# IRMVLab/EfficientLO-Net

Hardware: AMD Instinct MI355X
Metric: frame-pairs/sec (KITTI 64x1800 range image) (higher is better)
Workload: dtype f32 (1x1 convolutions as 3 fp16-MFMA products of hi/lo-split fp32 operands, fp32 accumulate)

## Files before the change

efficientlo-net_amd/csrc/elo_features.hip:

```cpp
#include <type_traits>
#include "elo_common.h"
#include "elo_project_device.h"

namespace elo {
namespace {

constexpr int ROWS_PER_BLOCK = ELO_BLOCK / ELO_WAVE;

__device__ __forceinline__ long row_of_wave(long total_rows)
{
    const long r = (long)xcd_tile(blockIdx.x, gridDim.x) * ROWS_PER_BLOCK + threadIdx.x / ELO_WAVE;
    return r < total_rows ? r : -1;
}

inline unsigned grid_for_rows(long rows) { return (unsigned)((rows + ROWS_PER_BLOCK - 1) / ROWS_PER_BLOCK); }

constexpr int STAGE_ROWS = 64;

__device__ __forceinline__ void stream_out(const float *tile, float *__restrict__ dst, long first_row, long rows, int CT)
{
    const long valid = (rows - first_row < STAGE_ROWS ? rows - first_row : STAGE_ROWS) * CT;
    float *o = dst + first_row * CT;
    const long vec = valid >> 2;
    for (long i = threadIdx.x; i < vec; i += ELO_BLOCK)
// ... 698 lines not shown
};

struct RowsByBeams {
    const float *mid;
    int half;
    __device__ __forceinline__ int cell(float at, float z, float r, int H, int W, float az_res) const
    {
        const float PI_F = 3.14159265358979323846f;
        const float c = (PI_F - at) / az_res;
        int col = c != c ? 0 : (int)c;
        const float s = z / r;
        int row = 0;
        for (int step = half; step >= 1; step >>= 1) row += !(s >= mid[row + step - 1]) ? step : 0;
        row = row > H - 1 ? H - 1 : row;
        col = col < 0 ? 0 : col > W - 1 ? W - 1 : col;
        return row * W + col;
    }
};

template <class Rows>
__device__ __forceinline__ void bin_point_by(float x, float y, float z, long i, int b, int H, int W, float az_res, const Rows &rows,
                                             const ProjScratch &ps)
{
    const float r = sqrtf(x * x + y * y + z * z);
    const float at = atan2f(y, x);
    const int cell = rows.cell(at, z, r, H, W, az_res);
    const unsigned rb = __float_as_uint(r);
    ps.cell_of[i] = cell;
    ps.rbits[i] = rb;
    if (rb == 0) {
        const int flag = b * ZFLAGS + zero_kind(at);
        const unsigned long long zeros = __ballot(1);
        const int leader = __ffsll((long long)zeros) - 1;
        if ((int)(threadIdx.x & 63) == leader || flag != __shfl(flag, leader)) ps.zflag[flag] = 0u;
        return;
    }
    unsigned *slot = ps.minr + (long)b * H * W + cell;
    if (__hip_atomic_load(slot, __ATOMIC_RELAXED, __HIP_MEMORY_SCOPE_AGENT) > rb) atomicMin(slot, rb);
}

__device__ __forceinline__ void bin_point(float x, float y, float z, long i, int b, int H, int W, float az_res, float vert_res,
                                          float vert_off, const ProjScratch &ps)
{
    bin_point_by(x, y, z, i, b, H, W, az_res, RowsByFormula{vert_res, vert_off}, ps);
}

__device__ __forceinline__ void warp_cell_point(const elo_warp_project_args &a, long i, int b, const float *q, const float *t,
                                                const ProjScratch &ps)
{
    float x = a.xyz[i * 3 + 0], y = a.xyz[i * 3 + 1], z = a.xyz[i * 3 + 2];
    if (q) {
        const bool keep = !(x == 0.0f && y == 0.0f && z == 0.0f);
        const float q0 = q[0], q1 = q[1], q2 = q[2], q3 = q[3];
        const float v0 = q0 * 0.0f - q1 * x - q2 * y - q3 * z;
        const float v1 = q0 * x + q1 * 0.0f + q2 * z - q3 * y;
        const float v2 = q0 * y - q1 * z + q2 * 0.0f + q3 * x;
        const float v3 = q0 * z + q1 * y - q2 * x + q3 * 0.0f;
        const float n2 = q0 * q0 + q1 * q1 + q2 * q2 + q3 * q3 + 1e-10f;
        const float i0 = q0 / n2, i1 = -q1 / n2, i2 = -q2 / n2, i3 = -q3 / n2;
        const float w1 = v0 * i1 + v1 * i0 + v2 * i3 - v3 * i2;
        const float w2 = v0 * i2 - v1 * i3 + v2 * i0 + v3 * i1;
        const float w3 = v0 * i3 + v1 * i2 - v2 * i1 + v3 * i0;
        const float k = keep ? 1.0f : 0.0f;
        x = (w1 + t[0]) * k; y = (w2 + t[1]) * k; z = (w3 + t[2]) * k;
        a.warped[i * 3 + 0] = x; a.warped[i * 3 + 1] = y; a.warped[i * 3 + 2] = z;
    }
    bin_point(x, y, z, i, b, a.H, a.W, a.az_res, a.vert_res, a.vert_off, ps);
}

__device__ __forceinline__ void hamilton(const float *a, const float *b, float *r)
{
    r[0] = a[0] * b[0] - a[1] * b[1] - a[2] * b[2] - a[3] * b[3];
    r[1] = a[0] * b[1] + a[1] * b[0] + a[2] * b[3] - a[3] * b[2];
    r[2] = a[0] * b[2] - a[1] * b[3] + a[2] * b[0] + a[3] * b[1];
    r[3] = a[0] * b[3] + a[1] * b[2] - a[2] * b[1] + a[3] * b[0];
}

__device__ __forceinline__ void normalise_q(const float *q, float *o)
{
    const float n = sqrtf(q[0] * q[0] + q[1] * q[1] + q[2] * q[2] + q[3] * q[3] + 1e-10f) + 1e-10f;
    for (int i = 0; i < 4; ++i) o[i] = q[i] / n;
}

#ifdef ELO_POSE_CLOCK
__device__ unsigned long long g_pose_clock[4 * 8 + 1];
#define POSE_STAMP(i) do { if (blockIdx.x == 0 && blockIdx.y == 0 && threadIdx.x == 0) {                                    \
        if ((i) == 0) pose_slot = (int)(g_pose_clock[32]++ % 4);                                                          \
        g_pose_clock[pose_slot * 8 + (i)] = __builtin_readcyclecounter(); } } while (0)
#else
#define POSE_STAMP(i) do { } while (0)
#endif

template <int BLOCK>
__global__ __launch_bounds__(BLOCK) void pose_head_kernel(const elo_pose_head_args a, const int parts,
                                                          const elo_warp_project_args w, const int with_warp)
{
    extern __shared__ float sm[];
    float *feat = sm, *big = sm + a.C, *head = big + a.hidden;
    const int b = blockIdx.y, tid = threadIdx.x;
    const SvPartials s = sv_partials(a.scratch, gridDim.y, a.C);
#ifdef ELO_POSE_CLOCK
    int pose_slot = 0;
#endif
    POSE_STAMP(0);
    constexpr int HEAD_C = 64;
    const bool model_head = a.C == HEAD_C && a.hidden == BLOCK;
    float wb[HEAD_C], wq[4], wt[3], bias_big = 0.0f;
    auto request_weights = [&]() {
        const int j = tid;
#pragma unroll
        for (int c = 0; c < HEAD_C; ++c) wb[c] = a.W_big[(size_t)c * a.hidden + j];
#pragma unroll
        for (int o = 0; o < 4; ++o) wq[o] = a.W_q[(size_t)j * 4 + o];
#pragma unroll
        for (int o = 0; o < 3; ++o) wt[o] = a.W_t[(size_t)j * 3 + o];
        bias_big = a.b_big[j];
    };
    float *mpart = head + 8 + 8 * (BLOCK / ELO_WAVE);
    if (model_head) request_weights();
    const int c = tid & 63, q = tid >> 6;
    float M = -INFINITY, D = 0.0f, A = 0.0f;
    if (c < a.C) {
        auto trips = [&](auto mine) {
            constexpr int MINE = decltype(mine)::value;
            for (int i0 = q; i0 < parts; i0 += 4 * MINE) {
                float m_[MINE], d_[MINE], a_[MINE];
#pragma unroll
                for (int u = 0; u < MINE; ++u) {
                    const int i = i0 + 4 * u;
                    const size_t at = ((size_t)b * ELO_SV_MAX_PARTS + (i < parts ? i : 0)) * a.C + c;
                    m_[u] = s.mx[at]; a_[u] = s.acc[at];
                    d_[u] = i < parts ? s.den[at] : 0.0f;
                }
#pragma unroll
                for (int u = 0; u < MINE; ++u) {
                    if (d_[u] == 0.0f) continue;
                    if (m_[u] > M) { const float sc = exp_acc(M - m_[u]); D = D * sc + d_[u]; A = A * sc + a_[u]; M = m_[u]; }
                    else { const float sc = exp_acc(m_[u] - M); D += d_[u] * sc; A += a_[u] * sc; }
                }
            }
        };
        if (parts <= 64) trips(std::integral_constant<int, 16>());
        else trips(std::integral_constant<int, 32>());
    }
    POSE_STAMP(1);
    mpart[(0 * 4 + q) * 64 + c] = M; mpart[(1 * 4 + q) * 64 + c] = D; mpart[(2 * 4 + q) * 64 + c] = A;
    __syncthreads();
    if (tid < 64) {
        float MM = -INFINITY;
        for (int i = 0; i < 4; ++i) MM = fmaxf(MM, mpart[(0 * 4 + i) * 64 + tid]);
        float DD = 0.0f, AA = 0.0f;
        for (int i = 0; i < 4; ++i) {
            if (mpart[(1 * 4 + i) * 64 + tid] == 0.0f) continue;
            const float sc = exp_acc(mpart[(0 * 4 + i) * 64 + tid] - MM);
            DD += mpart[(1 * 4 + i) * 64 + tid] * sc; AA += mpart[(2 * 4 + i) * 64 + tid] * sc;
        }
        if (tid < a.C) feat[tid] = DD > 0.0f ? AA / DD : 0.0f;
    }
    for (int c2 = 64 + tid; c2 < a.C; c2 += blockDim.x) feat[c2] = sv_merge(s, b, c2, a.C, parts);

    __syncthreads();
    POSE_STAMP(2);
    if (model_head) {
        float v = bias_big;
#pragma unroll
        for (int c = 0; c < HEAD_C; ++c) v += feat[c] * wb[c];
        big[tid] = v;
    } else {
        for (int j = tid; j < a.hidden; j += blockDim.x) {
            float v = a.b_big[j];
#pragma unroll 16
            for (int c = 0; c < a.C; ++c) v += feat[c] * a.W_big[(size_t)c * a.hidden + j];
            big[j] = v;
        }
    }
    __syncthreads();
    POSE_STAMP(3);
    {
        float part[7] = {0, 0, 0, 0, 0, 0, 0};
        if (model_head) {
            const float bj = big[tid];
#pragma unroll
            for (int o = 0; o < 4; ++o) part[o] += bj * wq[o];
#pragma unroll
            for (int o = 0; o < 3; ++o) part[4 + o] += bj * wt[o];
        } else {
            for (int j = tid; j < a.hidden; j += blockDim.x) {
                const float bj = big[j];
#pragma unroll
                for (int o = 0; o < 4; ++o) part[o] += bj * a.W_q[(size_t)j * 4 + o];
#pragma unroll
                for (int o = 0; o < 3; ++o) part[4 + o] += bj * a.W_t[(size_t)j * 3 + o];
            }
        }
#pragma unroll
        for (int o = 0; o < 7; ++o)
            for (int d = 32; d >= 1; d >>= 1) part[o] += __shfl_xor(part[o], d, ELO_WAVE);
        float *wsum = head + 8;
        if ((tid & 63) == 0)
            for (int o = 0; o < 7; ++o) wsum[(tid >> 6) * 8 + o] = part[o];
        __syncthreads();
        if (tid < 7) {
            float v = tid < 4 ? a.b_q[tid] : a.b_t[tid - 4];
            for (int w = 0; w < (int)(blockDim.x >> 6); ++w) v += wsum[w * 8 + tid];
            head[tid] = v;
        }
    }
    __syncthreads();
    POSE_STAMP(4);
    if (tid == 0) {
        float q_det[4], q[4], t[3], qn[4];
        normalise_q(head, q_det);
        const float *t_det = head + 4;
        if (a.q_coarse) {
            const float *qc = a.q_coarse + b * 4, *tc = a.t_coarse + b * 3;
            const float tq[4] = {0.0f, tc[0], tc[1], tc[2]};
            float v[4], w[4], inv[4];
            hamilton(q_det, tq, v);
            const float n2 = q_det[0] * q_det[0] + q_det[1] * q_det[1] + q_det[2] * q_det[2] + q_det[3] * q_det[3] + 1e-10f;
            inv[0] = q_det[0] / n2; inv[1] = -q_det[1] / n2; inv[2] = -q_det[2] / n2; inv[3] = -q_det[3] / n2;
            hamilton(v, inv, w);
            hamilton(q_det, qc, q);
            for (int i = 0; i < 3; ++i) t[i] = w[i + 1] + t_det[i];
        } else {
            for (int i = 0; i < 4; ++i) q[i] = q_det[i];
            for (int i = 0; i < 3; ++i) t[i] = t_det[i];
        }
        normalise_q(q, qn);
        if (blockIdx.x == 0) {
            for (int i = 0; i < 4; ++i) { a.q[b * 4 + i] = q[i]; a.q_norm[b * 4 + i] = qn[i]; }
            for (int i = 0; i < 3; ++i) a.t[b * 3 + i] = t[i];
            if (a.pose7) {
                float *row = a.pose7 + b * 7;
                if (a.pose7_slots > 1 && a.pose7_cursor) {
                    const unsigned at = a.pose7_cursor[b];
                    a.pose7_cursor[b] = at + 1u;
                    row += (size_t)(at % (unsigned)a.pose7_slots) * a.batch * 7;
                }
                for (int i = 0; i < 4; ++i) row[i] = qn[i];
                for (int i = 0; i < 3; ++i) row[4 + i] = t[i];
            }
        }
        if (with_warp) {
            for (int i = 0; i < 4; ++i) head[8 + i] = q[i];
            for (int i = 0; i < 3; ++i) head[12 + i] = t[i];
        }
    }
    POSE_STAMP(5);
    if (a.next_orders.pool && blockIdx.x == 0 && blockIdx.y == 0) perm_refresh_block(a.next_orders);
    POSE_STAMP(6);
    if (!with_warp) return;
    __syncthreads();
    const long n = (long)blockIdx.x * blockDim.x + tid;
    if (n < w.npoints) {
        warp_cell_point(w, (long)b * w.npoints + n, b, head + 8, head + 12,
                        proj_scratch(w.scratch, (size_t)w.batch * w.H * w.W, w.batch, (size_t)w.batch * w.npoints));
    }
    POSE_STAMP(7);
}

__global__ __launch_bounds__(ELO_BLOCK) void project_init_kernel(unsigned *minr, float *out_xyz, unsigned *out_feat,
                                                                 size_t cells, int C, int images)
{
    const size_t n_xyz = cells * 3, n_feat = cells * (size_t)C, total = cells + n_xyz + n_feat;
    for (size_t i = (size_t)blockIdx.x * blockDim.x + threadIdx.x; i < (size_t)images * ZFLAGS; i += (size_t)gridDim.x * blockDim.x)
        minr[cells + i] = 0x7f7f7f7fu;
    for (size_t i = (size_t)blockIdx.x * blockDim.x + threadIdx.x; i < total; i += (size_t)gridDim.x * blockDim.x) {
        if (i < cells) minr[i] = 0x7f7f7f7fu;
        else if (i < cells + n_xyz) out_xyz[i - cells] = 0.0f;
        else out_feat[i - cells - n_xyz] = 0u;
    }
}

__global__ __launch_bounds__(ELO_BLOCK) void warp_cell_kernel(const elo_warp_project_args a, const ProjScratch ps)
{
    const long total = (long)a.batch * a.npoints;
    for (long i = (long)blockIdx.x * blockDim.x + threadIdx.x; i < total; i += (long)gridDim.x * blockDim.x) {
        const int b = point_batch(i, a.npoints);
        warp_cell_point(a, i, b, a.q ? a.q + b * 4 : nullptr, a.q ? a.t + b * 3 : nullptr, ps);
    }
// ... 606 lines not shown
```

efficientlo-net_amd/csrc/elo_fused.hip:

```cpp
#include "elo_group_device.h"
#include "elo_project_device.h"
#include <atomic>
#include <cstdlib>
#include <type_traits>

namespace elo {
namespace {

typedef float f32x4 __attribute__((ext_vector_type(4)));
typedef _Float16 half4 __attribute__((ext_vector_type(4)));
typedef _Float16 half2v __attribute__((ext_vector_type(2)));

constexpr int FUSED_BLOCK = 256;
constexpr int FUSED_WAVES = 4;
__device__ __forceinline__ int ftid() { return (int)(threadIdx.x & (FUSED_BLOCK - 1)); }

constexpr int MODE_SPLIT = 0;
constexpr int MODE_HALF = 1;
constexpr int MODE_CHECKED = 2;

__device__ unsigned long long g_range_violations;
__device__ unsigned long long g_range_snapshot;
__global__ void range_take_kernel() { g_range_snapshot = atomicExch(&g_range_violations, 0ull); }

// ... 1016 lines not shown
        seg_store<TILE, MODE>(act, S, 0, w0, f16, r0, row_of, all, bad);
        if (w1) seg_store<TILE, MODE>(act, S, w0, w1, f16, r1, row_of, all, bad);
        if (w2) seg_store<TILE, MODE>(act, S, w0 + w1, w2, f16, r2, row_of, all, bad);
        zero_cols<TILE, MODE>(act, S, CT, CTp);
    } else {
        for (int e = tid; e < TILE * CTp; e += FUSED_BLOCK) {
            const int row = small_div(e, CTp), ch = e - row * CTp;
            const long gr = first + row;
            float v = 0.0f;
            if (gr < end && ch < CT) {
                v = ch < w0 ? feat_load(a.src[0], gr * w0 + ch, f16)
                  : ch < w0 + w1 ? feat_load(a.src[1], gr * w1 + (ch - w0), f16)
                                 : feat_load(a.src[2], gr * w2 + (ch - w0 - w1), f16);
            }
            act_put<MODE>(act, row * S + ch, v, bad);
        }
    }
    __syncthreads();
    const int N = a.layers[a.n_layers - 1].N;
    const bool two = a.n_layers2 > 0;
    for (int l = 0; l < a.n_layers; ++l)
        dense<TILE, MODE>(act, S, 0, a.layers[l],
                          l == a.n_layers - 1 ? LayerOut{two || keep_final ? 0 : -1, !two && keep_final ? 1 : 0, a.out, first, end, f16} : to_tile(0), bad);
    if (!two) return;
    const int wb = a.w_before, wa = a.w_after, CT2 = N + wb + wa;
    if ((N & 3) == 0 && (wb == 0 || seg_ok(a.before, wb, TILE, f16)) && (wa == 0 || seg_ok(a.after, wa, TILE, f16))) {
        uint4 rb[SEG_ITEMS], ra[SEG_ITEMS];
        if (wb) seg_load<TILE>(rb, a.before, wb, f16, row_of);
        if (wa) seg_load<TILE>(ra, a.after, wa, f16, row_of);
        if (wb) seg_store<TILE, MODE>(act, S, N, wb, f16, rb, row_of, all, bad);
        if (wa) seg_store<TILE, MODE>(act, S, N + wb, wa, f16, ra, row_of, all, bad);
    } else {
        for (int e = tid; e < TILE * (wb + wa); e += FUSED_BLOCK) {
            const int row = small_div(e, wb + wa), ch = e - row * (wb + wa);
            const long gr = first + row;
            const long grc = gr < end ? gr : end - 1;
            const float v = ch < wb ? feat_load(a.before, grc * wb + ch, f16) : feat_load(a.after, grc * wa + (ch - wb), f16);
            act_put<MODE>(act, row * S + N + ch, gr < end ? v : 0.0f, bad);
        }
    }
    zero_cols<TILE, MODE>(act, S, CT2, ceil16(CT2));
    __syncthreads();
    for (int l = 0; l < a.n_layers2; ++l)
        dense<TILE, MODE>(act, S, 0, a.layers2[l],
                          l == a.n_layers2 - 1 ? LayerOut{keep_final ? 0 : -1, keep_final ? 1 : 0, a.out2, first, end, f16} : to_tile(0), bad);
}

template <int TILE, int MODE>
__global__ __launch_bounds__(FUSED_BLOCK, TILE == 32 ? ELO_TILE32_WAVES : ELO_TILE_WAVES) void mlp_kernel(const JobPair<elo_mlp_args> jobs, const int S)
{
    const elo_mlp_args &a = jobs.job[blockIdx.y];
    extern __shared__ __align__(16) float lds[];
    unsigned bad = 0;
    {
        const elo_mlp_args &j0 = jobs.job[0];
        clear_projection(ProjectionClear{j0.clear_scratch, j0.clear_xyz, (unsigned *)j0.clear_feat, j0.clear_cells,
                                         j0.feat_dtype == ELO_F16 ? j0.clear_C / 2 : j0.clear_C, j0.clear_images});
    }
    const long first = (long)xcd_tile(blockIdx.x, gridDim.x) * TILE;
    if (first >= a.rows) return;
    mlp_tile<TILE, MODE>(a, lds, S, first, a.rows, false, bad);
    report_violations<MODE>(bad, a.range_counter);
}

template <int TILE, int MODE, bool PAIR>
__global__ __launch_bounds__(PAIR ? 2 * FUSED_BLOCK : FUSED_BLOCK, TILE == 32 ? 4 : ELO_TILE_WAVES)
void mlp_sv_kernel(const JobPair<elo_mlp_args> jobs, const int S, const int tiles_pb)
{
    constexpr int C = 64;
    const int group = PAIR ? __builtin_amdgcn_readfirstlane(threadIdx.x >> 8) : 0;
    const elo_mlp_args &j0 = jobs.job[0];
    const elo_mlp_args &a = jobs.job[group];
    extern __shared__ __align__(16) float lds[];
    const int tile_words = TILE * S;
    float *act = lds + group * tile_words;
    float *staged = lds + (PAIR ? 2 : 1) * tile_words;
    unsigned bad = 0;
    clear_projection(ProjectionClear{j0.clear_scratch, j0.clear_xyz, (unsigned *)j0.clear_feat, j0.clear_cells,
                                     j0.feat_dtype == ELO_F16 ? j0.clear_C / 2 : j0.clear_C, j0.clear_images});
    const unsigned tile = xcd_tile(blockIdx.x, gridDim.x);
    const int b = (int)(tile / (unsigned)tiles_pb), t = (int)(tile - (unsigned)b * (unsigned)tiles_pb);
    const long first = (long)b * j0.sv_npoints + (long)t * TILE, end = (long)(b + 1) * j0.sv_npoints;
    const int f16 = j0.feat_dtype == ELO_F16;
    const int vr = threadIdx.x < TILE ? (int)threadIdx.x : 0;
    const long vrow = first + vr < end ? first + vr : end - 1;
    const float px = j0.sv_xyz[vrow * 3 + 0], py = j0.sv_xyz[vrow * 3 + 1], pz = j0.sv_xyz[vrow * 3 + 2];
    constexpr int STAGE = PAIR ? 1 : TILE / 16;
    uint4 held[STAGE];
    if constexpr (!PAIR) {
#pragma unroll
        for (int u = 0; u < STAGE; ++u) {
            const int e = (int)threadIdx.x + u * FUSED_BLOCK, fr = e >> 4, q = e & 15;
            const long grow = first + fr < end ? first + fr : end - 1;
            if (f16) { const uint2 h = reinterpret_cast<const uint2 *>(j0.sv_feature)[grow * (C / 4) + q]; held[u] = uint4{h.x, h.y, 0u, 0u}; }
            else held[u] = reinterpret_cast<const uint4 *>(j0.sv_feature)[grow * (C / 4) + q];
        }
    }
    mlp_tile<TILE, MODE>(a, act, S, first, end, true, bad);
    report_violations<MODE>(bad, a.range_counter);
    if constexpr (!PAIR) {
#pragma unroll
        for (int u = 0; u < STAGE; ++u) {
            const int e = (int)threadIdx.x + u * FUSED_BLOCK, fr = e >> 4, q = e & 15;
            float4 v;
            if (f16) {
                const half2v h0 = __builtin_bit_cast(half2v, held[u].x), h1 = __builtin_bit_cast(half2v, held[u].y);
                v = float4{(float)h0.x, (float)h0.y, (float)h1.x, (float)h1.y};
            } else {
                v = __builtin_bit_cast(float4, held[u]);
            }
            *reinterpret_cast<float4 *>(staged + fr * C + 4 * q) = v;
        }
        __syncthreads();
    }
    if (threadIdx.x >= C) return;
    const unsigned long long okm = __ballot((threadIdx.x < TILE) & (first + vr < end) & !((px == 0.0f) & (py == 0.0f) & (pz == 0.0f)));
    const int c = threadIdx.x;
    const float *logit = lds + c, *value = PAIR ? lds + tile_words + c : staged + c;
    const int vs = PAIR ? S : C;
    float M = -INFINITY, D = 0.0f, A = 0.0f;
#pragma unroll
    for (int r0 = 0; r0 < TILE; r0 += 16) {
        float l[16], v[16];
#pragma unroll
        for (int r = 0; r < 16; ++r) { l[r] = logit[(r0 + r) * S]; v[r] = value[(r0 + r) * vs]; }
        const unsigned ok = (unsigned)(okm >> r0) & 0xffffu;
        float bm = -INFINITY;
#pragma unroll
        for (int r = 0; r < 16; ++r) bm = (ok >> r & 1u) ? fmaxf(bm, l[r]) : bm;
        if (bm > -INFINITY) {
            float d16 = 0.0f, a16 = 0.0f;
#pragma unroll
            for (int r = 0; r < 16; ++r) {
                const float e = (ok >> r & 1u) ? exp_acc(l[r] - bm) : 0.0f;
                d16 += e;
                a16 += e * v[r];
            }
            const float m2 = fmaxf(M, bm), s0 = exp_acc(M - m2), s1 = exp_acc(bm - m2);
            D = D * s0 + d16 * s1;
            A = A * s0 + a16 * s1;
            M = m2;
        }
    }
    float *sc = j0.sv_scratch;
    const size_t n = (size_t)(gridDim.x / (unsigned)tiles_pb) * ELO_SV_MAX_PARTS * C;
    const size_t at = ((size_t)b * ELO_SV_MAX_PARTS + t) * C + c;
    sc[at] = M; sc[n + at] = D; sc[2 * n + at] = A;
}

__host__ __device__ __forceinline__ int cv1_feat_cols(int C)
{
    const int kp = (10 + 2 * C + 15) & ~15;
    return kp > 2 * C + 16 ? kp : 2 * C + 16;
}

__device__ __forceinline__ elo_dense kernarg_dense(size_t byte_offset)
{
    static_assert(sizeof(elo_dense) == 48, "three 16-byte scalar loads");
    typedef const __attribute__((address_space(4))) char *KernargBytes;
    typedef unsigned int Quad __attribute__((ext_vector_type(4)));
    typedef const __attribute__((address_space(4))) Quad *KernargQuads;
    KernargBytes p = (KernargBytes)__builtin_amdgcn_kernarg_segment_ptr() + byte_offset;
    asm volatile("" : "+s"(p));
    KernargQuads q = reinterpret_cast<KernargQuads>(p);
    struct Raw { Quad a, b, c; } raw = {q[0], q[1], q[2]};
    return __builtin_bit_cast(elo_dense, raw);
}
#define CV1_LAYER(field) kernarg_dense(offsetof(elo_cv1_args, field))

template <int TILE, int MODE, bool GROUP = true>
__device__ __forceinline__ void cv1_tile(const elo_cv1_args &a, const int S, float *lds, unsigned block, unsigned nblocks)
{
    float *act = lds;
    const TileMeta meta = tile_meta(lds, TILE, S);
    const int tid = threadIdx.x;
    const int K = a.K, P = TILE / K, C = a.C, f16 = a.feat_dtype == ELO_F16;
    unsigned bad = 0;
    const long total_points = (long)a.batch * a.npoints;
    const long first_point = (long)xcd_tile(block, nblocks) * P;
    if (first_point >= total_points) return;
    CV1_STAMP(0);
    if (GROUP && a.group.random_hw) {
        int *lds_off = reinterpret_cast<int *>(act);
        unsigned *scratch = reinterpret_cast<unsigned *>(lds_off + ((a.group.kernel_h * a.group.kernel_w + 3) & ~3));
        group_tile<TILE, true>(meta, lds_off, scratch, a.group, first_point, total_points, a.npoints, P, K, a.xyz1, a.H2,
                               a.W2, nullptr, a.xyz2, a.H2, a.W2, nullptr);
    } else {
        load_meta<TILE>(meta, first_point, total_points, P, K, a.idx, a.mask, a.H2, a.W2);
        __syncthreads();
    }
    CV1_STAMP(1);
    const int F = 128, G = F + 2 * C;
    {
        auto cell_of = [&](int row) { return (long)meta.cell[row]; };
        auto centre_of = [&](int row) { return meta.cell[row] >= 0 ? first_point + small_div(row, K) : -1L; };
        uint4 r1[SEG_ITEMS], r2[SEG_ITEMS];
        seg_load<TILE>(r1, a.feat1, C, f16, centre_of);
        seg_load<TILE>(r2, a.feat2, C, f16, cell_of);
        GeoRow gr;
        const bool grow = tid < TILE;
        const int gcell = grow ? meta.cell[tid] : -1;
        if (grow) gr = geo_load(a.xyz1 + (gcell >= 0 ? first_point + small_div(tid, K) : 0) * 3, a.xyz2 + (long)(gcell >= 0 ? gcell : 0) * 3);
        seg_store<TILE, MODE>(act, S, F, C, f16, r1, centre_of, [](int) { return true; }, bad);
        seg_store<TILE, MODE>(act, S, F + C, C, f16, r2, cell_of, [&](int row) { return meta.mask[row] != 0.0f; }, bad);
        if (grow) geo_store<MODE>(act, tid * S + G, gr, meta.mask[tid], gcell >= 0, bad);
        zero_cols<TILE, MODE>(act, S, G + 16, F + cv1_feat_cols(C));
    }
    Pre<Sub<TILE, 128>::TPW> p128;
    Pre<Sub<TILE, 64>::TPW> p64;
    const elo_dense cv0 = CV1_LAYER(cv0);
    prefetch<TILE, Sub<TILE, 128>::TPW, MODE>(cv0, p128);
    __syncthreads();
    CV1_STAMP(2);
    const elo_dense cv1 = CV1_LAYER(cv1);
    dense_pf<TILE, 128, 64, MODE>(act, S, F, to_tile(0), cv0, p128, &cv1, &p64, bad);
    CV1_STAMP(3);
    const elo_dense cv2 = CV1_LAYER(cv2);
    dense_pf<TILE, 64, 64, MODE>(act, S, 0, to_tile(0), cv1, p64, &cv2, &p64, bad);
    CV1_STAMP(4);
    const elo_dense cv_xyz = CV1_LAYER(cv_xyz);
    dense_pf<TILE, 64, 64, MODE>(act, S, 0, to_tile(0), cv2, p64, &cv_xyz, &p64, bad);
    CV1_STAMP(5);
    const elo_dense sum_cv0 = CV1_LAYER(sum_cv0);
    dense_pf<TILE, 64, 128, MODE>(act, S, G, to_tile(64), cv_xyz, p64, &sum_cv0, &p128, bad);
    CV1_STAMP(6);
// ... 1532 lines not shown
    ELO_REQUIRE(!a->clear_scratch || a->clear_cells * (a->clear_C > 3 ? a->clear_C : 3) < (1l << 31), who, "clear_* side job: more than 2^31 words");
    ELO_REQUIRE(a->n_layers2 >= 0 && a->n_layers2 <= ELO_MAX_CHAIN, who, "0..3 second-stage layers");
    if (a->n_layers2 > 0) {
        ELO_REQUIRE(a->out2 && a->w_before >= 0 && a->w_after >= 0 && (a->before || a->w_before == 0) &&
                    (a->after || a->w_after == 0), who, "incomplete second stage");
        ELO_REQUIRE(width % 4 == 0, who, "a second stage needs a first-stage output width that is a multiple of 4");
        width += a->w_before + a->w_after;
        for (int l = 0; l < a->n_layers2; ++l) {
            if (int rc = check_dense(a->layers2[l], width, 0, who, "mlp stage 2")) return rc;
            width = a->layers2[l].N;
        }
    }
    return ELO_OK;
}

static int mlp_cols(const elo_mlp_args *a, int in_width)
{
    int cols = chain_cols(a->layers, a->n_layers, in_width);
    if (a->n_layers2 > 0) {
        const int n1 = a->layers[a->n_layers - 1].N, in2 = a->w_before + n1 + a->w_after;
        const int c2 = chain_cols(a->layers2, a->n_layers2, in2);
        cols = cols > c2 ? cols : c2;
    }
    return cols;
}

static bool mlp_chain_regime(long rows, bool pair, int batch_hint, int mode)
{
#ifdef ELO_DENSE_F32
    (void)rows; (void)pair; (void)batch_hint; (void)mode;
    return false;
#else
    return (mode == MODE_SPLIT || mode == MODE_HALF) && cv1_rr_on() && rows * (pair ? 2 : 1) >= mlp_rr_rows(batch_hint);
#endif
}

struct MlpPlan { int S, mode, C; bool t16, chain; int sv_tiles; size_t sv_lds; };

static int plan_mlp(const elo_mlp_args *a, const elo_mlp_args *b, MlpPlan *p, const char *who)
{
    int in_width = 0, in_width_b = 0;
    if (int rc = check_mlp(a, who, &in_width)) return rc;
    if (b) {
        if (int rc = check_mlp(b, who, &in_width_b)) return rc;
        bool same = a->rows == b->rows && in_width == in_width_b && a->n_layers == b->n_layers &&
                    a->n_layers2 == b->n_layers2 && a->w_before == b->w_before && a->w_after == b->w_after &&
                    a->feat_dtype == b->feat_dtype;
        for (int l = 0; same && l < a->n_layers; ++l) same = a->layers[l].N == b->layers[l].N;
        for (int l = 0; same && l < a->n_layers2; ++l) same = a->layers2[l].N == b->layers2[l].N;
        if (!same) return fail(ELO_ERR_ARG, "%s: the two jobs of a paired launch must have the same shape", who);
    }
    if (b && b->clear_scratch) return fail(ELO_ERR_ARG, "%s: the clear_* side job belongs to the first job of a pair", who);
    if (b && (b->sv_scratch || b->sv_feature)) return fail(ELO_ERR_ARG, "%s: the sv_* fields belong to the first job of a pair", who);
    p->S = row_stride(mlp_cols(a, in_width));
    const long u32 = (a->rows + 31) / 32;
    p->mode = 0;
    if (int rc = pair_products_mode(who, &p->mode, a->n_layers, a->n_layers2, a->layers, a->layers2, b ? b->layers : nullptr,
                                    b ? b->layers2 : nullptr))
        return rc;
    p->t16 = small_tile(u32 * (b ? 2 : 1), 1);
    p->chain = false;
    p->C = a->n_sources == 2 ? a->src_width[1] : 0;
#ifndef ELO_DENSE_F32
    {
        const int C = p->C;
        const auto aligned16 = [](const elo_mlp_args *j) {
            return ((uintptr_t)j->src[0] | (uintptr_t)j->src[1] | (uintptr_t)j->before | (uintptr_t)j->after | (uintptr_t)j->out |
                    (uintptr_t)j->out2) % 16 == 0;
        };
        const bool aligned = aligned16(a) && (!b || aligned16(b));
        p->chain = a->n_sources == 2 && a->src_width[0] == 64 &&
                   (C == 16 || C == 32 || C == 64) && a->n_layers == 2 && a->layers[0].N == 128 && a->layers[1].N == 64 && a->n_layers2 == 2 &&
                   a->layers2[0].N == 128 && a->layers2[1].N == 64 && a->w_before == C && a->w_after == 64 && aligned &&
                   mlp_chain_regime(a->rows, b != nullptr, a->batch_hint, p->mode);
    }
#endif
    p->sv_tiles = 0;
    p->sv_lds = 0;
    const int final_n = a->n_layers2 > 0 ? a->layers2[a->n_layers2 - 1].N : a->layers[a->n_layers - 1].N;
    if (!p->chain && final_n == 64 && a->sv_npoints > 0 && a->rows > 0 && a->rows % a->sv_npoints == 0) {
        const bool t16 = small_tile((a->rows / a->sv_npoints) * (((long)a->sv_npoints + 31) / 32), 1);
        const int tile = t16 ? 16 : 32, groups = b ? 2 : 1;
        const long tiles = ((long)a->sv_npoints + tile - 1) / tile;
        const size_t lds = sizeof(float) * ((size_t)groups * tile * p->S + (b ? 0 : (size_t)tile * 64));
        if (tiles <= ELO_SV_MAX_PARTS && lds <= 64 * 1024) {
            p->sv_tiles = (int)tiles;
            p->sv_lds = lds;
            p->t16 = t16;
        }
    }
    return ELO_OK;
}

extern "C" int elo_mlp_sv_parts(const elo_mlp_args *a, const elo_mlp_args *b)
{
    MlpPlan p;
    if (plan_mlp(a, b, &p, "elo_mlp_sv_parts")) return 0;
    return p.sv_tiles;
}

extern "C" int elo_mlp_fused2(const elo_mlp_args *a, const elo_mlp_args *b, elo_stream_t stream)
{
    const char *who = "elo_mlp_fused";
    MlpPlan plan;
    if (int rc = plan_mlp(a, b, &plan, who)) return rc;
    if (a->rows == 0)
        return a->clear_scratch || a->sv_scratch ? fail(ELO_ERR_ARG, "%s: a clear_* / sv_* side job needs rows to ride on", who) : ELO_OK;
    const int S = plan.S, mode = plan.mode;
    const bool t16 = plan.t16;
    const long u32 = (a->rows + 31) / 32, u16 = (a->rows + 15) / 16;
    JobPair<elo_mlp_args> pair;
    pair.job[0] = *a;
    pair.job[1] = b ? *b : *a;
    if (a->sv_scratch) {
        if (!plan.sv_tiles)
            return fail(ELO_ERR_ARG, "%s: sv_scratch is set but this launch cannot compute softmax_valid's partial sums "
                                     "(elo_mlp_sv_parts returns 0: chain-kernel regime, final width != 64, rows %% sv_npoints != 0 or too many tiles)", who);
        if (!a->sv_xyz) return fail(ELO_ERR_ARG, "%s: sv_scratch without sv_xyz", who);
        if ((b != nullptr) == (a->sv_feature != nullptr))
            return fail(ELO_ERR_ARG, "%s: a paired launch takes its features from job b (sv_feature NULL), a single launch from sv_feature", who);
        if (!b && ((uintptr_t)a->sv_feature & 15)) return fail(ELO_ERR_ARG, "%s: unaligned sv_feature", who);
        const size_t lds = plan.sv_lds;
        const dim3 grid((unsigned)(a->rows / a->sv_npoints) * (unsigned)plan.sv_tiles);
        hipStream_t s = (hipStream_t)stream;
#define CALL_SV(T_, M_)                                                                                                         \
        do {                                                                                                                    \
            if (b) hipLaunchKernelGGL((mlp_sv_kernel<T_, M_, true>), grid, dim3(2 * FUSED_BLOCK), lds, s, pair, S, plan.sv_tiles); \
            else hipLaunchKernelGGL((mlp_sv_kernel<T_, M_, false>), grid, dim3(FUSED_BLOCK), lds, s, pair, S, plan.sv_tiles);     \
        } while (0)
#define CALL_SV_T(M_, t16_) do { if (t16_) CALL_SV(16, M_); else CALL_SV(32, M_); } while (0)
        ELO_PICK_MODE(mode, CALL_SV_T, t16);
#undef CALL_SV_T
#undef CALL_SV
        ++g_sv_ride_launches;
        return check_launch(who);
    }
    const size_t lds = tile_lds_bytes(t16 ? 16 : 32, S);
#ifndef ELO_DENSE_F32
    if (plan.chain) {
        const dim3 rgrid((unsigned)((a->rows + RR_ROWS - 1) / RR_ROWS), b ? 2u : 1u);
        const bool f16 = a->feat_dtype == ELO_F16;
#define CALL(k) ELO_LAUNCH_RR(k, rgrid, (hipStream_t)stream, pair)
        ELO_PICK_RR_C(mlp2_rr_kernel, plan.C, f16, mode, CALL);
#undef CALL
        ++g_rr_launches[3];
        return check_launch(who);
    }
#endif
    const dim3 grid((unsigned)(t16 ? u16 : u32), b ? 2u : 1u);
    hipStream_t s = (hipStream_t)stream;
#define CALL(k) hipLaunchKernelGGL(k, grid, dim3(FUSED_BLOCK), lds, s, pair, S)
    ELO_PICK(mlp_kernel, t16, mode, CALL);
#undef CALL
    return check_launch(who);
}

extern "C" int elo_mlp_fused(const elo_mlp_args *a, elo_stream_t stream) { return elo_mlp_fused2(a, nullptr, stream); }

static int check_cv_features(const char *who, int C, int f16, std::initializer_list<const void *> tensors)
{
    const int per = f16 ? 8 : 4;
    if (C % per != 0) return fail(ELO_ERR_LIMIT, "%s: C = %d must be a multiple of %d (%s feature storage)", who, C, per, f16 ? "fp16" : "fp32");
    if (32 * (C / per) > SEG_ITEMS * FUSED_BLOCK) return fail(ELO_ERR_LIMIT, "%s: C = %d too wide for the tile gather", who, C);
    for (const void *p : tensors)
        if ((uintptr_t)p & 15) return fail(ELO_ERR_ARG, "%s: feature tensors must be 16-byte aligned", who);
    return ELO_OK;
}
// ... 261 lines not shown
```

Baseline: 12690.

## Parallelize softmax-pool tile reduction across waves and restructure pose-head merge

In the fused MLP softmax-pool epilogue, every wave now reduces a strided subset of tile rows per channel and writes (max, denom, acc) partials to LDS. One wave then merges those partials, where before a single wave walked every row serially. The pose head's partial merge first computes a block-wide channel max through LDS so each part is scaled once, with no running online rescaling. Its wave sums now use DPP row-rotate steps instead of a full shfl_xor tree. This adds an extra barrier and more LDS per block, which could affect occupancy.

```diff
diff --git a/efficientlo-net_amd/csrc/elo_features.hip b/efficientlo-net_amd/csrc/elo_features.hip
--- a/efficientlo-net_amd/csrc/elo_features.hip
+++ b/efficientlo-net_amd/csrc/elo_features.hip
@@ -804,6 +804,21 @@
     for (int i = 0; i < 4; ++i) o[i] = q[i] / n;
 }
 
+__device__ __forceinline__ float wave_sum_xor_tree(float v)
+{
+    const auto add = [](float x, float y) { return x + y; };
+    const auto ror = [](float x, auto ctrl) {
+        const int u = (int)__float_as_uint(x);
+        return x + __uint_as_float((unsigned)__builtin_amdgcn_update_dpp(u, u, decltype(ctrl)::value, 0xf, 0xf, false));
+    };
+    v = bfly<32>(v, add);
+    v = bfly<16>(v, add);
+    v = bfly<8>(v, add);
+    v = ror(v, std::integral_constant<int, 0x124>());
+    v = ror(v, std::integral_constant<int, 0x122>());
+    return ror(v, std::integral_constant<int, 0x121>());
+}
+
 #ifdef ELO_POSE_CLOCK
 __device__ unsigned long long g_pose_clock[4 * 8 + 1];
 #define POSE_STAMP(i) do { if (blockIdx.x == 0 && blockIdx.y == 0 && threadIdx.x == 0) {                                    \
@@ -840,44 +855,82 @@
     };
     float *mpart = head + 8 + 8 * (BLOCK / ELO_WAVE);
     if (model_head) request_weights();
-    const int c = tid & 63, q = tid >> 6;
-    float M = -INFINITY, D = 0.0f, A = 0.0f;
-    if (c < a.C) {
-        auto trips = [&](auto mine) {
-            constexpr int MINE = decltype(mine)::value;
-            for (int i0 = q; i0 < parts; i0 += 4 * MINE) {
-                float m_[MINE], d_[MINE], a_[MINE];
-#pragma unroll
-                for (int u = 0; u < MINE; ++u) {
-                    const int i = i0 + 4 * u;
-                    const size_t at = ((size_t)b * ELO_SV_MAX_PARTS + (i < parts ? i : 0)) * a.C + c;
-                    m_[u] = s.mx[at]; a_[u] = s.acc[at];
-                    d_[u] = i < parts ? s.den[at] : 0.0f;
-                }
-#pragma unroll
-                for (int u = 0; u < MINE; ++u) {
-                    if (d_[u] == 0.0f) continue;
-                    if (m_[u] > M) { const float sc = exp_acc(M - m_[u]); D = D * sc + d_[u]; A = A * sc + a_[u]; M = m_[u]; }
-                    else { const float sc = exp_acc(m_[u] - M); D += d_[u] * sc; A += a_[u] * sc; }
-                }
+    const int c = tid & 63, q = tid >> 6, cc = c < a.C ? c : a.C - 1;
+    const auto slot = [&](int i) { return ((size_t)b * ELO_SV_MAX_PARTS + (i < parts ? i : 0)) * a.C + cc; };
+    const auto channel_max = [&](float mine) {
+        mpart[q * 64 + c] = mine;
+        __syncthreads();
+        return fmaxf(fmaxf(mpart[0 * 64 + c], mpart[1 * 64 + c]), fmaxf(mpart[2 * 64 + c], mpart[3 * 64 + c]));
+    };
+    float D = 0.0f, A = 0.0f;
+    const auto held = [&](auto mine) {
+        constexpr int MINE = decltype(mine)::value;
+        float m_[MINE], d_[MINE], a_[MINE];
+#pragma unroll
+        for (int u = 0; u < MINE; ++u) {
+            const int i = q + 4 * u;
+            m_[u] = s.mx[slot(i)];
+            d_[u] = i < parts ? s.den[slot(i)] : 0.0f;
+        }
+#pragma unroll
+        for (int u = 0; u < MINE; ++u) a_[u] = s.acc[slot(q + 4 * u)];
+        float lm = -INFINITY;
+#pragma unroll
+        for (int u = 0; u < MINE; ++u) {
+            const bool live = d_[u] != 0.0f;
+            m_[u] = live ? m_[u] : -INFINITY; a_[u] = live ? a_[u] : 0.0f;
+            lm = fmaxf(lm, m_[u]);
+        }
+        const float MM = channel_max(lm);
+#pragma unroll
+        for (int u = 0; u < MINE; ++u) {
+            const float sc = exp_acc(m_[u] - MM);
+            D += d_[u] * sc;
+            A += a_[u] * sc;
+        }
+    };
+    const auto reread = [&]() {
+        constexpr int MAXES = 32, SUMS = 16;
+        float lm = -INFINITY;
+        for (int i0 = q; i0 < parts; i0 += 4 * MAXES) {
+            float m_[MAXES], d_[MAXES];
+#pragma unroll
+            for (int u = 0; u < MAXES; ++u) {
+                const int i = i0 + 4 * u;
+                m_[u] = s.mx[slot(i)];
+                d_[u] = i < parts ? s.den[slot(i)] : 0.0f;
             }
-        };
-        if (parts <= 64) trips(std::integral_constant<int, 16>());
-        else trips(std::integral_constant<int, 32>());
-    }
+#pragma unroll
+            for (int u = 0; u < MAXES; ++u) lm = d_[u] != 0.0f ? fmaxf(lm, m_[u]) : lm;
+        }
+        const float MM = channel_max(lm);
+        for (int i0 = q; i0 < parts; i0 += 4 * SUMS) {
+            float m_[SUMS], d_[SUMS], a_[SUMS];
+#pragma unroll
+            for (int u = 0; u < SUMS; ++u) {
+                const int i = i0 + 4 * u;
+                m_[u] = s.mx[slot(i)]; a_[u] = s.acc[slot(i)];
+                d_[u] = i < parts ? s.den[slot(i)] : 0.0f;
+            }
+#pragma unroll
+            for (int u = 0; u < SUMS; ++u) {
+                const bool live = d_[u] != 0.0f;
+                const float sc = exp_acc((live ? m_[u] : -INFINITY) - MM);
+                D += d_[u] * sc;
+                A += (live ? a_[u] : 0.0f) * sc;
+            }
+        }
+    };
+    if (parts <= 64) held(std::integral_constant<int, 16>());
+    else if (parts <= 128) held(std::integral_constant<int, 32>());
+    else reread();
     POSE_STAMP(1);
-    mpart[(0 * 4 + q) * 64 + c] = M; mpart[(1 * 4 + q) * 64 + c] = D; mpart[(2 * 4 + q) * 64 + c] = A;
+    mpart[(1 * 4 + q) * 64 + c] = D; mpart[(2 * 4 + q) * 64 + c] = A;
     __syncthreads();
-    if (tid < 64) {
-        float MM = -INFINITY;
-        for (int i = 0; i < 4; ++i) MM = fmaxf(MM, mpart[(0 * 4 + i) * 64 + tid]);
-        float DD = 0.0f, AA = 0.0f;
-        for (int i = 0; i < 4; ++i) {
-            if (mpart[(1 * 4 + i) * 64 + tid] == 0.0f) continue;
-            const float sc = exp_acc(mpart[(0 * 4 + i) * 64 + tid] - MM);
-            DD += mpart[(1 * 4 + i) * 64 + tid] * sc; AA += mpart[(2 * 4 + i) * 64 + tid] * sc;
-        }
-        if (tid < a.C) feat[tid] = DD > 0.0f ? AA / DD : 0.0f;
+    if (tid < 64 && tid < a.C) {
+        const float *dp = mpart + 1 * 4 * 64 + tid, *ap = mpart + 2 * 4 * 64 + tid;
+        const float DD = (dp[0 * 64] + dp[1 * 64]) + (dp[2 * 64] + dp[3 * 64]), AA = (ap[0 * 64] + ap[1 * 64]) + (ap[2 * 64] + ap[3 * 64]);
+        feat[tid] = DD > 0.0f ? AA / DD : 0.0f;
     }
     for (int c2 = 64 + tid; c2 < a.C; c2 += blockDim.x) feat[c2] = sv_merge(s, b, c2, a.C, parts);
 
@@ -916,8 +969,7 @@
             }
         }
 #pragma unroll
-        for (int o = 0; o < 7; ++o)
-            for (int d = 32; d >= 1; d >>= 1) part[o] += __shfl_xor(part[o], d, ELO_WAVE);
+        for (int o = 0; o < 7; ++o) part[o] = wave_sum_xor_tree(part[o]);
         float *wsum = head + 8;
         if ((tid & 63) == 0)
             for (int o = 0; o < 7; ++o) wsum[(tid >> 6) * 8 + o] = part[o];
diff --git a/efficientlo-net_amd/csrc/elo_fused.hip b/efficientlo-net_amd/csrc/elo_fused.hip
--- a/efficientlo-net_amd/csrc/elo_fused.hip
+++ b/efficientlo-net_amd/csrc/elo_fused.hip
@@ -1122,7 +1122,10 @@
     const int b = (int)(tile / (unsigned)tiles_pb), t = (int)(tile - (unsigned)b * (unsigned)tiles_pb);
     const long first = (long)b * j0.sv_npoints + (long)t * TILE, end = (long)(b + 1) * j0.sv_npoints;
     const int f16 = j0.feat_dtype == ELO_F16;
-    const int vr = threadIdx.x < TILE ? (int)threadIdx.x : 0;
+    constexpr int NW = (PAIR ? 2 : 1) * FUSED_WAVES, RPW = TILE / NW;
+    float *part = staged + (PAIR ? 0 : TILE * C);
+    const int lane = (int)(threadIdx.x & 63u), wave = __builtin_amdgcn_readfirstlane((int)(threadIdx.x >> 6));
+    const int vr = lane < TILE ? lane : 0;
     const long vrow = first + vr < end ? first + vr : end - 1;
     const float px = j0.sv_xyz[vrow * 3 + 0], py = j0.sv_xyz[vrow * 3 + 1], pz = j0.sv_xyz[vrow * 3 + 2];
     constexpr int STAGE = PAIR ? 1 : TILE / 16;
@@ -1153,34 +1156,37 @@
         }
         __syncthreads();
     }
+    const unsigned long long okm = __ballot((lane < TILE) & (first + vr < end) & !((px == 0.0f) & (py == 0.0f) & (pz == 0.0f)));
+    {
+        const float *logit = lds + lane, *value = PAIR ? lds + tile_words + lane : staged + lane;
+        const int vs = PAIR ? S : C;
+        float l[RPW], v[RPW];
+#pragma unroll
+        for (int k = 0; k < RPW; ++k) { l[k] = logit[(wave + k * NW) * S]; v[k] = value[(wave + k * NW) * vs]; }
+        float bm = -INFINITY;
+#pragma unroll
+        for (int k = 0; k < RPW; ++k) bm = (okm >> (wave + k * NW) & 1ull) ? fmaxf(bm, l[k]) : bm;
+        float d = 0.0f, a_ = 0.0f;
+#pragma unroll
+        for (int k = 0; k < RPW; ++k) {
+            const float e = (okm >> (wave + k * NW) & 1ull) ? exp_acc(l[k] - bm) : 0.0f;
+            d += e;
+            a_ += e * v[k];
+        }
+        part[(wave * 3 + 0) * C + lane] = bm; part[(wave * 3 + 1) * C + lane] = d; part[(wave * 3 + 2) * C + lane] = a_;
+    }
+    __syncthreads();
     if (threadIdx.x >= C) return;
-    const unsigned long long okm = __ballot((threadIdx.x < TILE) & (first + vr < end) & !((px == 0.0f) & (py == 0.0f) & (pz == 0.0f)));
     const int c = threadIdx.x;
-    const float *logit = lds + c, *value = PAIR ? lds + tile_words + c : staged + c;
-    const int vs = PAIR ? S : C;
     float M = -INFINITY, D = 0.0f, A = 0.0f;
 #pragma unroll
-    for (int r0 = 0; r0 < TILE; r0 += 16) {
-        float l[16], v[16];
-#pragma unroll
-        for (int r = 0; r < 16; ++r) { l[r] = logit[(r0 + r) * S]; v[r] = value[(r0 + r) * vs]; }
-        const unsigned ok = (unsigned)(okm >> r0) & 0xffffu;
-        float bm = -INFINITY;
-#pragma unroll
-        for (int r = 0; r < 16; ++r) bm = (ok >> r & 1u) ? fmaxf(bm, l[r]) : bm;
-        if (bm > -INFINITY) {
-            float d16 = 0.0f, a16 = 0.0f;
-#pragma unroll
-            for (int r = 0; r < 16; ++r) {
-                const float e = (ok >> r & 1u) ? exp_acc(l[r] - bm) : 0.0f;
-                d16 += e;
-                a16 += e * v[r];
-            }
-            const float m2 = fmaxf(M, bm), s0 = exp_acc(M - m2), s1 = exp_acc(bm - m2);
-            D = D * s0 + d16 * s1;
-            A = A * s0 + a16 * s1;
-            M = m2;
-        }
+    for (int w = 0; w < NW; ++w) M = fmaxf(M, part[(w * 3 + 0) * C + c]);
+#pragma unroll
+    for (int w = 0; w < NW; ++w) {
+        const float d = part[(w * 3 + 1) * C + c];
+        const float sc = d == 0.0f ? 0.0f : exp_acc(part[(w * 3 + 0) * C + c] - M);
+        D += d * sc;
+        A += part[(w * 3 + 2) * C + c] * sc;
     }
     float *sc = j0.sv_scratch;
     const size_t n = (size_t)(gridDim.x / (unsigned)tiles_pb) * ELO_SV_MAX_PARTS * C;
@@ -2879,7 +2885,7 @@
         const bool t16 = small_tile((a->rows / a->sv_npoints) * (((long)a->sv_npoints + 31) / 32), 1);
         const int tile = t16 ? 16 : 32, groups = b ? 2 : 1;
         const long tiles = ((long)a->sv_npoints + tile - 1) / tile;
-        const size_t lds = sizeof(float) * ((size_t)groups * tile * p->S + (b ? 0 : (size_t)tile * 64));
+        const size_t lds = sizeof(float) * ((size_t)groups * tile * p->S + (b ? 0 : (size_t)tile * 64) + (size_t)groups * FUSED_WAVES * 3 * 64);
         if (tiles <= ELO_SV_MAX_PARTS && lds <= 64 * 1024) {
             p->sv_tiles = (int)tiles;
             p->sv_lds = lds;
```

Measured after the change: 12470. 0.983x the previous value.
